# sbrodeur/hierarchical-sparse-coding

Measured on NVIDIA B200. Metric: mp_atoms_per_s, higher is better.
Workload: dtype f32

## Files before the change

### hierarchical_sparse_coding_b200/csrc/engine.cu

```cuda
#include <cuda_runtime.h>
#include <stdio.h>
#include <stdlib.h>
#include <string.h>
#include <math.h>

#include <string>
#include <vector>

#include "../../include/hsc_b200.h"
#include "common.cuh"
#include "correlate_simt.cuh"
#include "correlate_tc.cuh"
#include "pursuit.cuh"
#include "locomp.cuh"
#include "decode.cuh"
#include "ksvd.cuh"
#include "kmeans.cuh"
#include "events.cuh"

using namespace hsc;

namespace {

size_t align_up(size_t v, size_t a = 256) { return (v + a - 1) / a * a; }
// ... 272 lines not shown
    a.has_snr = !isnan(e->opt.tolerance_snr); a.tol_snr = a.has_snr ? (real)e->opt.tolerance_snr : (real)0;
    a.has_scale = !isnan(e->opt.tolerance_residual_scale);
    a.tol_scale = a.has_scale ? (real)e->opt.tolerance_residual_scale : (real)0;
    a.null_thres = (real)e->opt.min_coefficients;
    a.eps = sizeof(real) == 4 ? (real)1.1920928955078125e-07 : (real)2.220446049250313e-16;
    if (e->opt.energy_eps > 0.0) a.eps = (real)e->opt.energy_eps;
    a.coef_mode = e->opt.coef_mode;
    a.max_passes = e->opt.max_passes_per_run;
    a.max_events_total = e->opt.max_events_total;
    a.nb_blocks = e->opt.nb_blocks;
    a.ncand_max = l.ncand_max;
    a.edge_ext = (real*)(e->ws + l.off_edge); a.edge_stride = l.edge_stride;
    a.cand_t = (int*)(e->ws + l.off_cand_t); a.cand_k = (int*)(e->ws + l.off_cand_k); a.cand_c = (real*)(e->ws + l.off_cand_c);
    a.prof = nullptr;
    a.locomp_scratch = nullptr;
    {
        static const char* rr_env = getenv("HSC_RERANK");
        double tol = e->opt.rerank_tolerance < 0.0 ? 4e-6 : e->opt.rerank_tolerance;
        if (rr_env) tol = atof(rr_env);
        a.rerank_tol = sizeof(real) == 4 ? (float)tol : 0.f;
    }
    {
        static const int early = getenv("HSC_K2_EARLY_ISSUE") ? atoi(getenv("HSC_K2_EARLY_ISSUE")) : 0;
        a.early_issue = early > 0 ? 1 : 0;
        static const int nextpf = getenv("HSC_K2_NEXT_PREFETCH") ? atoi(getenv("HSC_K2_NEXT_PREFETCH")) : -1;
        a.next_prefetch = nextpf >= 0 ? (nextpf > 0 ? 1 : 0)
                                      : ((e->K * sizeof(real)) / 16 >= 32 && e->S > 1 && e->S <= 2 * 148 ? 1 : 0);
    }
    static const int prefetch = getenv("HSC_PREFETCH") ? atoi(getenv("HSC_PREFETCH")) : -1;
    a.prefetch = prefetch;
    static const int variant = getenv("HSC_PURSUIT_VARIANT") ? atoi(getenv("HSC_PURSUIT_VARIANT")) : 4;
    static const int tma_mode = getenv("HSC_K2_TMA") ? atoi(getenv("HSC_K2_TMA")) : 1;
    static const int tma_stages_max = getenv("HSC_K2_TMA_STAGES") ? atoi(getenv("HSC_K2_TMA_STAGES")) : 4;
    a.tma_rows = a.tma_stages = a.tma_bytes = 0;
    size_t dyn_smem = 0;
    int rps = 1;
    const size_t row_bytes = (size_t)e->K * sizeof(real);
    const int NW = variant == 6 ? 4 : 8;
    if (tma_mode && variant != 0 && row_bytes % 16 == 0) {
        const int VN = 16 / (int)sizeof(real);
        const int nvec = (int)e->K / VN;
        const int gv = nvec >= 32 ? 32 : pow2_at_least(nvec);
        const int W = 2 * (int)e->L - 1;
        const int rpw = 32 / gv;
        if (variant == 6 && (size_t)NW * 3 * 2 * 2 * rpw * row_bytes <= 48 * 1024 && W >= 2 * NW * 2 * rpw) rps = 2;
        const size_t stage = (size_t)NW * 2 * rpw * rps * row_bytes;
        const int steps = (W + NW * rpw * rps - 1) / (NW * rpw * rps);
        int ns = (int)((48 * 1024) / stage);
        if (ns < 2) ns = (int)((72 * 1024) / stage);
        if (ns < 3 && e->S <= 2 * 148) ns = (int)((100 * 1024) / stage) < 3 ? ns : 3;
        {
            static const int ring_kb = getenv("HSC_K2_RING_KB") ? atoi(getenv("HSC_K2_RING_KB")) : 0;
            if (ring_kb > 0) ns = (int)(((size_t)ring_kb * 1024) / stage);
        }
        if (ns > tma_stages_max) ns = tma_stages_max;
        if (ns > steps) ns = steps;
        if (ns > 32 / NW) ns = 32 / NW;
        if (ns >= 1) {
            a.tma_rows = rpw * rps; a.tma_stages = ns;
            dyn_smem = stage * ns;
            a.tma_bytes = (int)dyn_smem;
// ... 48 lines not shown
            }
        }
        if (!fast) {
            a.tma_rows = a.tma_stages = a.tma_bytes = 0;
            locomp_kernel<real, 128><<<(unsigned)e->S, 128, 0, st>>>(a);
        }
        e->launches++;
        HSC_CUDA(e, cudaGetLastError());
        return HSC_OK;
    }
    static const int smh_mode = getenv("HSC_K2_SMH") ? atoi(getenv("HSC_K2_SMH")) : 1;
    const bool slots_fit = l.n2 <= kSlotMax || (e->S <= 148 && dyn_smem + (size_t)l.n2 * sizeof(unsigned long long) + slot3_bytes <= 200 * 1024);
    const bool smh = (dyn_smem > 0 || tiny_row) && smh_mode && sizeof(real) == 4 && l.G1 == 128 && slots_fit && (l.G1 % 32) == 0 &&
                     (2 * e->L - 1 + l.G1 - 1) / l.G1 + 1 <= kDirtyMax && (long long)l.G1 * e->K < (1ll << 32);
    if (smh) dyn_smem += (size_t)l.n2 * sizeof(unsigned long long) + slot3_bytes;
    {
        static const int smem_kb = getenv("HSC_K2_SMEM_KB") ? atoi(getenv("HSC_K2_SMEM_KB")) : 0;
        if (smem_kb > 0 && dyn_smem > 0 && dyn_smem < (size_t)smem_kb * 1024) dyn_smem = (size_t)smem_kb * 1024;
    }
#define HSC_LAUNCH_K2(NT_, MINB_, VIF_, TMA_, SMH_, RPS_)                                                                        \
    do {                                                                                                                          \
        if (dyn_smem > 0)                                                                                                         \
            HSC_CUDA(e, cudaFuncSetAttribute(pursuit_kernel<real, NT_, MINB_, VIF_, TMA_, SMH_, RPS_>,                            \
                                             cudaFuncAttributeMaxDynamicSharedMemorySize, (int)dyn_smem));                        \
        pursuit_kernel<real, NT_, MINB_, VIF_, TMA_, SMH_, RPS_><<<(unsigned)e->S, NT_, dyn_smem, st>>>(a);                       \
    } while (0)
    switch (variant) {
        case 0:
            HSC_LAUNCH_K2(256, 2, 4, false, false, 1);
            break;
        case 6:
            if (dyn_smem > 0 && smh && rps == 2) HSC_LAUNCH_K2(128, 4, 2, true, true, 2);
            else if (dyn_smem > 0 && smh) HSC_LAUNCH_K2(128, 4, 2, true, true, 1);
            else if (dyn_smem > 0 && rps == 2) HSC_LAUNCH_K2(128, 4, 2, true, false, 2);
            else if (dyn_smem > 0) HSC_LAUNCH_K2(128, 4, 2, true, false, 1);
            else HSC_LAUNCH_K2(128, 4, 2, false, false, 1);
            break;
        default:
            if (tiny_row && smh) HSC_LAUNCH_K2(256, 4, 2, false, true, 1);
            else if (dyn_smem > 0 && smh) HSC_LAUNCH_K2(256, 4, 2, true, true, 1);
            else if (dyn_smem > 0) HSC_LAUNCH_K2(256, 4, 2, true, false, 1);
            else HSC_LAUNCH_K2(256, 4, 2, false, false, 1);
            break;
    }
#undef HSC_LAUNCH_K2
    e->launches++;
    HSC_CUDA(e, cudaGetLastError());
#ifdef HSC_PROFILE_PHASES
    {
        std::vector<long long> h((size_t)e->S * 16);
        cudaStreamSynchronize(st);
        cudaMemcpy(h.data(), a.prof, h.size() * sizeof(long long), cudaMemcpyDeviceToHost);
        double tot[8] = {0, 0, 0, 0, 0, 0, 0, 0};
        for (long long i = 0; i < e->S; ++i) for (int j = 0; j < 8; ++j) tot[j] += (double)h[(size_t)i * 16 + j];
// ... 850 lines not shown
```

### hierarchical_sparse_coding_b200/csrc/pursuit.cuh

```cuda
#pragma once
#include <limits.h>
#include "common.cuh"

namespace hsc {

template <typename real>
struct MpArgs {
    int T, K, L, F, off;
    int G1, n2, G2, n3;
    const real* D;
    const real* G;
    const real* w;
    real* map;
    real* resid;
    real* val1; int* idx1;
    real* val2; int* idx2;
    real* val3; int* idx3;
    unsigned* bitmap;
    long long bitmap_words;
    hsc_signal_state* state;
    int* ev_pos; int* ev_idx; real* ev_coef;
    long long cap;
    long long max_nnz;
    real tol_snr; int has_snr;
// ... 6 lines not shown
    int nb_blocks;
    int ncand_max;
    int* cand_t; int* cand_k; real* cand_c;
    double* locomp_scratch;
    real* edge_ext;
    long long edge_stride;
    int prefetch;
    int tma_rows, tma_stages;
    int tma_bytes;
    long long* prof;
    int scalar_window;
    int row32;
    int next_prefetch;
    int early_issue;
    float rerank_tol;
};

__device__ __forceinline__ unsigned long long pack_key(float v, int row_local, int k, int K) {
    const unsigned vb = __float_as_uint(v);
    return vb == 0u ? 0ull : (((unsigned long long)vb << 32) | (unsigned long long)(0xFFFFFFFFu - (unsigned)(row_local * K + k)));
}
__device__ __forceinline__ unsigned long long pack_key(double, int, int, int) { return 0ull; }

__device__ __forceinline__ unsigned lds_u32(uint32_t saddr) {
    unsigned v;
    asm("ld.shared.u32 %0, [%1];" : "=r"(v) : "r"(saddr));
    return v;
}

__device__ __forceinline__ unsigned long long warp_max_u64(unsigned long long key) {
// ... 422 lines not shown
                cur_key = 0ull;
            }
            cur_key = key > cur_key ? key : cur_key;
        }
        gmap += gstep;
        ggram += gstep;
        trow += NW;
        s = (s + 1 == NS) ? 0 : s + 1;
    }
    if constexpr (SMH) {
        if (lane == 0 && cur_key) atomicMax(&dirty[cur_g - glo], cur_key);
    }
    return phase;
}

template <typename real, int NT>
__device__ __noinline__ void edge_recorrelate(const MpArgs<real>& a, real* map_s, const real* ext, int ext_row0, int ra, int rb) {
    const int K = a.K, F = a.F, LF = a.L * a.F;
    constexpr int R = 8, U = 8;
    constexpr int KPT = NT <= 128 ? 2 : 1;
    const int kt = K < NT ? K : NT;
    const int ngroups = NT / kt;
    const int grp = threadIdx.x / kt;
    if (grp >= ngroups) return;
    const int nchunks = (rb - ra + 1 + R - 1) / R;
    for (int kk = threadIdx.x - grp * kt; kk < K; kk += KPT * kt) {
        const real* dd[KPT];
#pragma unroll
        for (int p = 0; p < KPT; ++p) dd[p] = a.D + (long long)min(kk + p * kt, K - 1) * LF;
        for (int c = grp; c < nchunks; c += ngroups) {
// ... 125 lines not shown

template <typename real>
__device__ __forceinline__ double exact_score_warp(const MpArgs<real>& a, const hsc_signal_state& st, const real* map_s, const real* res_s,
                                                   int r, int k) {
    double sc;
    const bool overhang = (r < a.off) || (r > a.T - a.L + a.off);
    if (!overhang || !overhang_row_written(st, r, a.off, a.T, a.L)) sc = fabs(residual_dot_warp<real>(a, res_s, r, k));
    else sc = fabs((double)__ldcg(map_s + (long long)r * a.K + k));
    return a.w ? sc * fabs((double)a.w[k]) : sc;
}

constexpr int kRerankMax = 32;

template <typename real, typename Lvl2>
__device__ __forceinline__ void rerank_candidates(const MpArgs<real>& a, const hsc_signal_state& st, const real* map_s, const real* res_s,
                                                  const real* v1, Lvl2 lvl2, uint32_t slot3_saddr, int g1s, real thr, int& t_out, int& k_out) {
    __shared__ int cand_g[kRerankMax], cand_r[kRerankMax], cand_k[kRerankMax];
    const int lane = threadIdx.x & 31;
    const int T = a.T, K = a.K, L = a.L, F = a.F, LF = a.L * a.F;
    int ng = 0;
    if (slot3_saddr) {
        const int n3 = (a.n2 + 31) >> 5;
        for (int b0 = 0; b0 < n3; b0 += 32) {
            const int b = b0 + lane;
            unsigned mb = __ballot_sync(0xffffffffu, b < n3 && (real)__uint_as_float(lds_u32(slot3_saddr + 4u * (unsigned)b)) >= thr);
            while (mb) {
                const int g = ((b0 + __ffs(mb) - 1) << 5) + lane;
                mb &= mb - 1;
                const bool h = g < a.n2 && lvl2(g) >= thr;
                const unsigned m = __ballot_sync(0xffffffffu, h);
                if (h) { const int slot = ng + __popc(m & ((1u << lane) - 1u)); if (slot < kRerankMax) cand_g[slot] = g; }
// ... 23 lines not shown
            for (int u = 0; u < 4; ++u) { const int r = rb + u * 32 + lane; h[u] = r < r_end && v1[r] >= thr; }
#pragma unroll
            for (int u = 0; u < 4; ++u) {
                const unsigned m = __ballot_sync(0xffffffffu, h[u]);
                if (h[u]) { const int slot = nr + __popc(m & ((1u << lane) - 1u)); if (slot < kRerankMax) cand_r[slot] = rb + u * 32 + lane; }
                nr += __popc(m);
            }
        }
    }
    nr = min(nr, kRerankMax);
    __syncwarp();
    int nc = 0;
    for (int i = 0; i < nr; ++i) {
        const int rr = cand_r[i];
        const real* mrow = map_s + (long long)rr * K;
        for (int kb = 0; kb < K; kb += 128) {
            bool h[4];
#pragma unroll
            for (int u = 0; u < 4; ++u) {
                const int kk = kb + u * 32 + lane;
                h[u] = false;
                if (kk < K) { const real m = __ldcg(mrow + kk); h[u] = rabs<real>(a.w ? m * a.w[kk] : m) >= thr; }
            }
#pragma unroll
            for (int u = 0; u < 4; ++u) {
                const unsigned m = __ballot_sync(0xffffffffu, h[u]);
                if (h[u]) {
                    const int slot = nc + __popc(m & ((1u << lane) - 1u));
                    if (slot < kRerankMax) { cand_g[slot] = rr; cand_k[slot] = kb + u * 32 + lane; }
                }
                nc += __popc(m);
            }
        }
    }
    nc = min(nc, kRerankMax);
    __syncwarp();
    const int sub = lane >> 3, sl = lane & 7;
// ... 29 lines not shown
        }
        for (int m = 16; m >= 8; m >>= 1) {
            const double os = __shfl_xor_sync(0xffffffffu, sc, m);
            const long long of = __shfl_xor_sync(0xffffffffu, flat, m);
            if (os > sc || (os == sc && of < flat)) { sc = os; flat = of; }
        }
        if (sc > best || (sc == best && flat < best_flat)) { best = sc; best_flat = flat; }
    }
    if (best_flat != LLONG_MAX && best >= 0.0) {
        t_out = (int)(best_flat / K);
        k_out = (int)(best_flat - (long long)t_out * K);
    }
}

template <typename real>
__device__ __forceinline__ bool near_tie_in_group(const MpArgs<real>& a, const real* map_s, const real* v1, int g1s, int t, int k, real thr) {
    const int lane = threadIdx.x & 31;
    bool amb = false;
    const int r0 = (t >> g1s) << g1s, r1 = min(r0 + (1 << g1s), a.T);
    const real* mrow = map_s + (long long)t * a.K;
    constexpr int RU = 4, MU = 8;
    real vv[RU], mm[MU];
#pragma unroll
    for (int u = 0; u < RU; ++u) { const int r = r0 + lane + 32 * u; vv[u] = r < r1 ? v1[r] : (real)-1; }
#pragma unroll
    for (int u = 0; u < MU; ++u) { const int kk = lane + 32 * u; mm[u] = kk < a.K ? __ldcg(mrow + kk) : (real)0; }
#pragma unroll
    for (int u = 0; u < RU; ++u) { const int r = r0 + lane + 32 * u; amb |= r < r1 && r != t && vv[u] >= thr; }
    for (int r = r0 + lane + 32 * RU; r < r1; r += 32) amb |= (r != t) && (v1[r] >= thr);
#pragma unroll
    for (int u = 0; u < MU; ++u) {
        const int kk = lane + 32 * u;
        amb |= kk < a.K && (kk != k) && (rabs<real>(a.w ? mm[u] * a.w[kk] : mm[u]) >= thr);
    }
    for (int kk = lane + 32 * MU; kk < a.K; kk += 32) {
        const real m = __ldcg(mrow + kk);
        amb |= (kk != k) && (rabs<real>(a.w ? m * a.w[kk] : m) >= thr);
    }
    return __any_sync(0xffffffffu, amb);
}

template <typename real, bool SMH>
__device__ __noinline__ real near_tie_watch(const MpArgs<real>& a, hsc_signal_state& st, const real* map_s, const real* res_s,
                                            const real* v1, const int* i1, const real* v2g, const real* v3g, const int* i3g, int g1s,
                                            int t, int k, real vbest, real second, uint32_t slot2_saddr, int next_g) {
    const int lane = threadIdx.x & 31;
    if constexpr (!SMH) {
        real bv = (real)0;
        int bt = INT_MAX;
        for (int e = lane; e < a.n3; e += 32) take_first_max(bv, bt, v3g[e], i3g[e]);
        group_argmax(bv, bt, 32);
        if (bt == INT_MAX) return (real)-1;
        t = bt;
        k = i1[t];
        vbest = bv;
    }
    if (st.reserved == 0) {
        __syncwarp();
        if (lane == 0) st.reserved = (int)__float_as_uint((float)vbest);
        __syncwarp();
    }
    const real thr = vbest - (real)a.rerank_tol * (vbest + (real)__uint_as_float((unsigned)st.reserved));
    bool amb;
    if constexpr (SMH) {
        amb = second >= thr;
    } else {
        const int gsel = t >> g1s;
        amb = false;
        for (int e = lane; e < a.n2; e += 32) amb |= (e != gsel) && (v2g[e] >= thr);
        amb = __any_sync(0xffffffffu, amb);
    }
    if (!amb) amb = near_tie_in_group<real>(a, map_s, v1, g1s, t, k, thr);
    if constexpr (SMH) {
        if (a.next_prefetch && next_g < 0 && second > (real)0) {
            const unsigned sbits = __float_as_uint((float)second);
            const uint32_t slot3_saddr = slot2_saddr + 8u * (unsigned)a.n2;
            const int n3 = (a.n2 + 31) >> 5;
            int bb = INT_MAX;
            for (int e = lane; e < n3; e += 32)
                if (lds_u32(slot3_saddr + 4u * (unsigned)e) == sbits && e != ((t >> g1s) >> 5)) bb = min(bb, e);
            bb = __reduce_min_sync(0xffffffffu, bb);
            if (bb != INT_MAX) {
                const int g = (bb << 5) + lane;
                const unsigned ghi = g < a.n2 ? lds_u32(slot2_saddr + 8u * (unsigned)g + 4u) : 0u;
                const int gg = __reduce_min_sync(0xffffffffu, ghi == sbits ? g : INT_MAX);
                if (gg != INT_MAX) next_g = gg;
            }
// ... 14 lines not shown
            } else {
                const int r0 = next_g << g1s;
                p = v1 + r0;
                bytes = (unsigned)(min(r0 + (1 << g1s), a.T) - r0) * sizeof(real);
            }
            if ((((unsigned long long)p) & 15ull) == 0 && (bytes & 15u) == 0 && bytes > 0)
                asm volatile("cp.async.bulk.prefetch.L2.global [%0], %1;" :: "l"(p), "r"(bytes) : "memory");
        }
    }
    return amb ? thr : (real)-1;
}

template <typename real, bool SMH>
__device__ __noinline__ real near_tie_resolve(const MpArgs<real>& a, hsc_signal_state& st, const real* map_s, const real* res_s,
                                              const real* v1, uint32_t slot2_saddr, const real* v2g, int g1s, real thr,
                                              int& t, int& k) {
    if constexpr (SMH) {
        auto lvl2 = [&](int g) { return (real)__uint_as_float(lds_u32(slot2_saddr + 8u * (unsigned)g + 4u)); };
        rerank_candidates<real>(a, st, map_s, res_s, v1, lvl2, slot2_saddr + 8u * (unsigned)a.n2, g1s, thr, t, k);
    } else {
        auto lvl2 = [&](int g) { return v2g[g]; };
        rerank_candidates<real>(a, st, map_s, res_s, v1, lvl2, 0u, g1s, thr, t, k);
    }
    const bool row_overhangs = (t < a.off) || (t > a.T - a.L + a.off);
    const bool from_residual = a.coef_mode == 1 && (!row_overhangs || !overhang_row_written(st, t, a.off, a.T, a.L));
    return from_residual ? (real)residual_dot_warp<real>(a, res_s, t, k) : __ldcg(map_s + (long long)t * a.K + k);
}

template <typename real, int NT>
__device__ __noinline__ int build_pass_list(const MpArgs<real>& a, const real* map_s, const real* res_s, const real* v1,
                                            const int* i1, int* ct, int* ck, real* cc, int offset_flag, double energy_signal) {
    const int T = a.T, K = a.K, L = a.L, F = a.F, off = a.off, LF = L * F;
    const int tid = threadIdx.x, lane = tid & 31, warp = tid >> 5, nwarps = NT >> 5;
    __shared__ int s_count;
    int bs = a.nb_blocks < 0 ? 4 * L : (int)floor((double)T / (double)a.nb_blocks);
    if (bs & 1) bs += 1;
    int nblk = (T + bs - 1) / bs;
// ... 132 lines not shown
        out[4] = g2 == INT_MAX ? -1 : g2;
    }
    __threadfence_block();
}

__device__ __forceinline__ void refold_block(const unsigned long long* slot2, unsigned* slot3, int b, int n2) {
    const int g = (b << 5) + (int)(threadIdx.x & 31);
    const unsigned hi = g < n2 ? (unsigned)(slot2[g] >> 32) : 0u;
    const unsigned mx = __reduce_max_sync(0xffffffffu, hi);
    if ((threadIdx.x & 31) == 0) slot3[b] = mx;
}

constexpr int kSlotMax = 1024;
constexpr int kDirtyMax = 8;

template <typename real, int NT, int MINB, int VIF, bool TMA, bool SMH, int RPS = 1>
__global__ void __launch_bounds__(NT, MINB) pursuit_kernel(MpArgs<real> a) {
    const int s = blockIdx.x;
    const int tid = threadIdx.x, lane = tid & 31, warp = tid >> 5;
    constexpr int NW = NT / 32;
    const int T = a.T, K = a.K, L = a.L, F = a.F, off = a.off;
    const int W = 2 * L - 1;
    const int LF = L * F;
#ifdef HSC_PROFILE_PHASES
    long long prof_kernel_t0;
    { unsigned long long ns_; asm volatile("mov.u64 %0, %%globaltimer;" : "=l"(ns_)); prof_kernel_t0 = (long long)ns_; }
#endif

    struct Ctx {
        real* map_s; real* res_s; real* v1; int* i1; real* v2; int* i2; real* v3; int* i3;
        unsigned* bits; int* evp; int* evi; real* evc;
        int* ct; int* ck; real* cc;
// ... 35 lines not shown
        real coef;
        real thr;
    } sel;
    __shared__ double red_a[NW], red_b[NW];
    __shared__ real red_m[NW];
    __shared__ struct { int t, k; unsigned vbest, second; int g2; } watch;

    extern __shared__ __align__(128) unsigned char win_smem[];
    __shared__ __align__(8) unsigned long long win_bar[(NT / 32) * 4];
    constexpr bool tma_on = TMA;
    unsigned win_phase = 0;
    unsigned long long* slot2 = reinterpret_cast<unsigned long long*>(win_smem + a.tma_bytes);
    unsigned* slot3 = reinterpret_cast<unsigned*>(slot2 + a.n2);
    __shared__ unsigned long long dirty_slot[kDirtyMax];
    const int g1s = 31 - __clz(a.G1);
    if (tid == 0) {
        st = a.state[s];
        if (tma_on) {
            for (int i = 0; i < (NT / 32) * a.tma_stages; ++i) mbarrier_init(smem_addr_u32(&win_bar[i]), 1);
            asm volatile("fence.mbarrier_init.release.cluster;" ::: "memory");
            fence_proxy_async_all();
        }
    }
    __syncthreads();
    if (st.status != HSC_RUNNING && st.status != HSC_PAUSE_CAPACITY && st.status != HSC_PAUSE_PASSES) return;

    const int g = min(32, pow2_at_least(K));
    const int ngroups = NT / g;
    const int grp = tid / g, lig = tid % g;
    constexpr int VN = VecOf<real>::N;
// ... 38 lines not shown
            st.initialised = 1;
        }
        if constexpr (!SMH) {
            rekey_level<real>(v1, nullptr, T, v2, i2, 0, a.n2 - 1, a.G1, NT);
            __syncthreads();
            rekey_level<real>(v2, i2, a.n2, v3, i3, 0, a.n3 - 1, a.G2, NT);
            __syncthreads();
        }
    }
    if constexpr (SMH) {
        if (tid < kDirtyMax) dirty_slot[tid] = 0ull;
        for (int gi = warp; gi < a.n2; gi += NW) {
            unsigned long long best = 0ull;
            const int e1 = min((gi + 1) << g1s, T);
            for (int r = (gi << g1s) + lane; r < e1; r += 32) {
                const unsigned long long key = pack_key(v1[r], r & (a.G1 - 1), i1[r], K);
                best = key > best ? key : best;
            }
            best = warp_max_u64(best);
            if (lane == 0) slot2[gi] = best;
        }
        __syncthreads();
        for (int b = warp; b < (a.n2 + 31) >> 5; b += NW) refold_block(slot2, slot3, b, a.n2);
    }
    if (tid == 0) {
        st.status = HSC_RUNNING;
        st.n_buffered = 0;
    }
    __syncthreads();

    long long passes_this_run = 0;
    const bool rerank_on = sizeof(real) == 4 && a.rerank_tol > 0.f && a.nb_blocks == 1;
#ifdef HSC_PROFILE_PHASES
    long long prof_t = clock64(), prof_acc[8] = {0, 0, 0, 0, 0, 0, 0, 0};
    long long prof_edge[4] = {0, 0, 0, 0};
    long long prof_loop_t0;
    { unsigned long long ns_; asm volatile("mov.u64 %0, %%globaltimer;" : "=l"(ns_)); prof_loop_t0 = (long long)ns_; }
#define HSC_STAMP(i) do { if (tid == 0) { long long now_ = clock64(); prof_acc[i] += now_ - prof_t; prof_t = now_; } } while (0)
#else
#define HSC_STAMP(i) do { } while (0)
#endif
    while (true) {
        HSC_STAMP(0);
        if (st.n_buffered >= a.cap) {
            if (tid == 0) st.status = HSC_PAUSE_CAPACITY;
            break;
        }
        const bool block_mode = a.nb_blocks != 1;
        const bool new_pass = !block_mode || st.pass_cursor >= st.pass_count;
        if (new_pass && a.max_passes > 0 && passes_this_run >= a.max_passes) {
            if (tid == 0) st.status = HSC_PAUSE_PASSES;
            break;
        }
        if (block_mode && new_pass) {
            const int n = build_pass_list<real, NT>(a, map_s, res_s, v1, i1, cx.ct, cx.ck, cx.cc, st.offset_flag, st.energy_signal);
            if (tid == 0) {
                st.pass_count = n;
                st.pass_cursor = 0;
            }
            __syncthreads();
            if (n == 0) {
                if (tid == 0) {
                    st.passes += 1;
                    st.status = HSC_STOP_EMPTY;
                }
// ... 64 lines not shown
            if constexpr (SMH) {
                asm volatile("bar.sync 1, 64;" ::: "memory");
                if (watch.t >= 0)
                    thr = near_tie_watch<real, true>(a, st, map_s, res_s, v1, i1, v2, v3, i3, g1s, watch.t, watch.k,
                                                     (real)__uint_as_float(watch.vbest), (real)__uint_as_float(watch.second),
                                                     smem_addr_u32(slot2), watch.g2);
            } else {
                thr = near_tie_watch<real, false>(a, st, map_s, res_s, v1, i1, v2, v3, i3, g1s, 0, 0, (real)0, (real)-1, 0u, -1);
            }
            if (lane == 0) sel.thr = thr;
        }
        __syncthreads();
        if (rerank_on && sel.thr >= (real)0) {
            if (warp == 0) {
                int t = sel.t, k = sel.k;
                const real coef = near_tie_resolve<real, SMH>(a, st, map_s, res_s, v1, smem_addr_u32(slot2), v2, g1s, sel.thr, t, k);
                __syncwarp();
                if (lane == 0) {
                    sel.t = t;
                    sel.k = k;
                    sel.edge = (t - (L - 1) < off) || (t + (L - 1) > T - L + off);
                    sel.coef = coef;
                    st.reranked += 1;
                }
            }
            __syncthreads();
        }
        HSC_STAMP(1);
        const int t = sel.t, k = sel.k, edge = sel.edge;
        const real coef = sel.coef;
        const bool pass_ends = sel.last != 0;

        const bool is_null = (a.null_thres >= (real)0) ? !(rabs<real>(coef) > a.null_thres) : (coef == (real)0);
        if (!block_mode && is_null) {
            if (tid == 0) {
                st.passes += 1;
                st.status = HSC_STOP_EMPTY;
            }
            break;
        }

        if constexpr (TMA) {
            if (!edge && a.early_issue) gram_window_issue<real, NT, RPS>(K, L, map_s, a.G + (long long)k * W * K, t, gv, win_smem, win_bar, a.tma_stages);
        }

        unsigned bk_old = 0u, bk_m = 0u;
        if (tid == 0) {
            const unsigned long long bit = (unsigned long long)t * K + k;
            bk_m = 1u << (bit & 31);
            bk_old = atomicOr(bits + (bit >> 5), bk_m);
            evp[st.n_buffered] = t;
            evi[st.n_buffered] = k;
            evc[st.n_buffered] = coef;
            st.n_buffered += 1;
            st.n_events += 1;
        }
        HSC_STAMP(5);

// ... 4 lines not shown
        const int jhi = (sstart + L > T) ? (T - sstart) : L;
        const real* dd = a.D + (long long)k * LF;
        real* rr = res_s + (long long)sstart * F;
        const int q_first = jlo * F + tid;
        real ro_first = (real)0, dq_first = (real)0;
        if (q_first < jhi * F) {
            ro_first = rr[q_first];
            dq_first = dd[q_first];
        }

        if constexpr (SMH) {
            const int span0 = g2_lo << g1s, span1 = min((g2_hi + 1) << g1s, T);
            for (int r0 = span0 + warp * 32; r0 < span1; r0 += NT) {
                const int r = r0 + lane;
                unsigned long long key = 0ull;
                if (r < span1 && (r < row_lo || r > row_hi)) key = pack_key(v1[r], r & (a.G1 - 1), i1[r], K);
                key = warp_max_u64(key);
                if (lane == 0 && key) atomicMax(&dirty_slot[(r0 >> g1s) - g2_lo], key);
            }
        }

        {
            double eb = 0.0, ea = 0.0;
            if (q_first < jhi * F) {
                const real rn = sub_scaled(ro_first, coef, dq_first);
                rr[q_first] = rn;
                eb = fma((double)ro_first, (double)ro_first, eb);
                ea = fma((double)rn, (double)rn, ea);
            }
            for (int q = q_first + NT; q < jhi * F; q += NT) {
                real ro = rr[q];
// ... 2 lines not shown
                eb = fma((double)ro, (double)ro, eb);
                ea = fma((double)rn, (double)rn, ea);
            }
            eb = warp_sum(eb);
            ea = warp_sum(ea);
            if (lane == 0) {
                red_b[warp] = eb;
                red_a[warp] = ea;
            }
        }
        HSC_STAMP(6);

        if (!edge) {
            const real* Gk = a.G + (long long)k * W * K;
            if constexpr (TMA) {
                if (!a.early_issue) gram_window_issue<real, NT, RPS>(K, L, map_s, Gk, t, gv, win_smem, win_bar, a.tma_stages);
                if (a.w) win_phase = gram_update_tma<real, NT, true, SMH, RPS>(K, L, a.w, map_s, Gk, v1, i1, t, coef, gv, win_smem, win_bar, a.tma_stages, win_phase, dirty_slot, g2_lo, g1s, true);
                else if (RPS == 1 && gv == 32 && a.row32) win_phase = gram_update_row32<real, NT, SMH>(K, L, map_s, Gk, v1, i1, t, coef, win_smem, win_bar, a.tma_stages, win_phase, dirty_slot, g2_lo, g1s);
                else win_phase = gram_update_tma<real, NT, false, SMH, RPS>(K, L, a.w, map_s, Gk, v1, i1, t, coef, gv, win_smem, win_bar, a.tma_stages, win_phase, dirty_slot, g2_lo, g1s, true);
            }
            else if (!(SMH && !TMA) && vec_pv == 1 && !a.w && !a.scalar_window) gram_update_vec<real, 1, NT, VIF, false>(K, L, a.w, map_s, Gk, v1, i1, t, coef, gv);
            else if (!(SMH && !TMA) && vec_pv == 2 && !a.w && !a.scalar_window) gram_update_vec<real, 2, NT, VIF, false>(K, L, a.w, map_s, Gk, v1, i1, t, coef, gv);
            else if (!(SMH && !TMA) && vec_pv == 4 && VIF >= 4 && !a.w && !a.scalar_window) gram_update_vec<real, 4, NT, VIF, false>(K, L, a.w, map_s, Gk, v1, i1, t, coef, gv);
            else {
                for (int base = 0; base < W; base += ngroups) {
                    const int i = base + grp;
                    const bool valid = i < W;
                    real bv = (real)0;
                    int bi = INT_MAX;
                    const int tr = t - (L - 1) + i;
                    if (valid) {
                        real* mrow = map_s + (long long)tr * K;
                        const real* grow = Gk + (long long)i * K;
                        for (int kk = lig; kk < K; kk += g) {
// ... 71 lines not shown
                    slot2[g2_lo + lane] = dirty_slot[lane];
                    dirty_slot[lane] = 0ull;
                }
                __syncwarp();
                for (int b = g2_lo >> 5; b <= g2_hi >> 5; ++b) refold_block(slot2, slot3, b, a.n2);
            }
        } else {
            rekey_level<real>(v1, nullptr, T, v2, i2, g2_lo, g2_hi, a.G1, NT);
        }
        if (tid == 0) {
            double eb = 0.0, ea = 0.0;
            for (int i = 0; i < NW; ++i) {
                eb += red_b[i];
                ea += red_a[i];
            }
            if (bk_old & bk_m) st.duplicates += 1;
            else st.nnz += 1;
            const real loss = (real)eb - (real)ea;
            const real e_now = (real)st.energy_residual - loss;
            st.energy_residual = (double)e_now;
            if (block_mode) st.pass_cursor += 1;
            int stop = 0;
            if (e_now < a.eps) {
                stop = HSC_STOP_ENERGY;
            } else {
                const real snr = (real)10 * rlog10<real>((real)st.energy_signal / e_now);
                if (a.max_nnz >= 0 && st.nnz >= a.max_nnz) stop = HSC_STOP_NNZ;
                else if (a.has_snr && snr >= a.tol_snr) stop = HSC_STOP_SNR;
                else if (a.max_events_total > 0 && st.n_events >= a.max_events_total) stop = HSC_STOP_MAX_EVENTS;
            }
// ... 57 lines not shown
#undef HSC_STAMP
#undef map_s
#undef res_s
#undef v1
#undef i1
#undef v2
#undef i2
#undef v3
#undef i3
#undef bits
#undef evp
#undef evi
#undef evc
}

}
```

Baseline: 10.30 million.

## Add lazy read-only correlation map path deferring interior Gram updates via event log

Adds a lazy pursuit kernel variant in which interior map rows are no longer written back after each atom selection. Selected atoms are logged, and when a window is loaded their contributions are reapplied on the fly through an extra TMA-loaded Gram row, plus direct loads for further overlapping events. Only band rows near the signal edges are stored. The log is flushed to global memory when there are too many overlaps or when the run pauses, and runner-up values are saved so tie detection still works. The aim is to remove per-iteration global write-back traffic, at the cost of extra Gram reads, a larger staging ring and considerable added complexity.

```diff
diff --git a/hierarchical_sparse_coding_b200/csrc/engine.cu b/hierarchical_sparse_coding_b200/csrc/engine.cu
--- a/hierarchical_sparse_coding_b200/csrc/engine.cu
+++ b/hierarchical_sparse_coding_b200/csrc/engine.cu
@@ -310,6 +310,8 @@
     a.cand_t = (int*)(e->ws + l.off_cand_t); a.cand_k = (int*)(e->ws + l.off_cand_k); a.cand_c = (real*)(e->ws + l.off_cand_c);
     a.prof = nullptr;
     a.locomp_scratch = nullptr;
+    a.lazy = 0;
+    a.runner = (unsigned*)(e->ws + l.off_keys);
     {
         static const char* rr_env = getenv("HSC_RERANK");
         double tol = e->opt.rerank_tolerance < 0.0 ? 4e-6 : e->opt.rerank_tolerance;
@@ -333,6 +335,11 @@
     int rps = 1;
     const size_t row_bytes = (size_t)e->K * sizeof(real);
     const int NW = variant == 6 ? 4 : 8;
+    const char* ro_env = getenv("HSC_K2_READONLY_MAP");
+    const bool lazy_shape = (!ro_env || atoi(ro_env) != 0) && sizeof(real) == 4 && e->opt.method == 0 && variant == 4 && tma_mode && !(e->opt.use_weights && e->w_dev) &&
+                            e->opt.nb_blocks == 1 && e->opt.coef_mode == 1 && e->T <= 65536 && (e->K * sizeof(real)) / 16 >= 32 &&
+                            (size_t)e->K * (2 * e->L - 1) * e->K * sizeof(real) <= 64ull * 1024 * 1024;
+    const int stage_rows = lazy_shape ? 3 : 2;
     if (tma_mode && variant != 0 && row_bytes % 16 == 0) {
         const int VN = 16 / (int)sizeof(real);
         const int nvec = (int)e->K / VN;
@@ -340,7 +347,7 @@
         const int W = 2 * (int)e->L - 1;
         const int rpw = 32 / gv;
         if (variant == 6 && (size_t)NW * 3 * 2 * 2 * rpw * row_bytes <= 48 * 1024 && W >= 2 * NW * 2 * rpw) rps = 2;
-        const size_t stage = (size_t)NW * 2 * rpw * rps * row_bytes;
+        const size_t stage = (size_t)NW * stage_rows * rpw * rps * row_bytes;
         const int steps = (W + NW * rpw * rps - 1) / (NW * rpw * rps);
         int ns = (int)((48 * 1024) / stage);
         if (ns < 2) ns = (int)((72 * 1024) / stage);
@@ -419,6 +426,10 @@
     const bool smh = (dyn_smem > 0 || tiny_row) && smh_mode && sizeof(real) == 4 && l.G1 == 128 && slots_fit && (l.G1 % 32) == 0 &&
                      (2 * e->L - 1 + l.G1 - 1) / l.G1 + 1 <= kDirtyMax && (long long)l.G1 * e->K < (1ll << 32);
     if (smh) dyn_smem += (size_t)l.n2 * sizeof(unsigned long long) + slot3_bytes;
+    if (lazy_shape && smh && a.row32 && a.tma_stages >= 1 && (size_t)a.tma_bytes >= (size_t)kLazyLogCap * 8 && l.n2 <= kSlotMax) {
+        a.lazy = 1;
+        dyn_smem += kLazySmemBytes;
+    }
     {
         static const int smem_kb = getenv("HSC_K2_SMEM_KB") ? atoi(getenv("HSC_K2_SMEM_KB")) : 0;
         if (smem_kb > 0 && dyn_smem > 0 && dyn_smem < (size_t)smem_kb * 1024) dyn_smem = (size_t)smem_kb * 1024;
@@ -442,7 +453,12 @@
             else HSC_LAUNCH_K2(128, 4, 2, false, false, 1);
             break;
         default:
-            if (tiny_row && smh) HSC_LAUNCH_K2(256, 4, 2, false, true, 1);
+            if (a.lazy && sizeof(real) == 4) {
+                const MpArgs<float>& af = reinterpret_cast<const MpArgs<float>&>(a);
+                HSC_CUDA(e, cudaFuncSetAttribute(pursuit_kernel_ro<256, 4>, cudaFuncAttributeMaxDynamicSharedMemorySize, (int)dyn_smem));
+                pursuit_kernel_ro<256, 4><<<(unsigned)e->S, 256, dyn_smem, st>>>(af);
+            }
+            else if (tiny_row && smh) HSC_LAUNCH_K2(256, 4, 2, false, true, 1);
             else if (dyn_smem > 0 && smh) HSC_LAUNCH_K2(256, 4, 2, true, true, 1);
             else if (dyn_smem > 0) HSC_LAUNCH_K2(256, 4, 2, true, false, 1);
             else HSC_LAUNCH_K2(256, 4, 2, false, false, 1);
diff --git a/hierarchical_sparse_coding_b200/csrc/pursuit.cuh b/hierarchical_sparse_coding_b200/csrc/pursuit.cuh
--- a/hierarchical_sparse_coding_b200/csrc/pursuit.cuh
+++ b/hierarchical_sparse_coding_b200/csrc/pursuit.cuh
@@ -44,6 +44,8 @@
     int next_prefetch;
     int early_issue;
     float rerank_tol;
+    int lazy;
+    unsigned* runner;
 };
 
 __device__ __forceinline__ unsigned long long pack_key(float v, int row_local, int k, int K) {
@@ -496,6 +498,286 @@
     return phase;
 }
 
+constexpr int kLazyBand = 3;
+constexpr int kLazyLogCap = 768;
+constexpr int kLazyOvMax = 16;
+constexpr int kLazySmemBytes = 16 + kLazyLogCap * 2 + kLazyOvMax * 16;
+constexpr int kLazyRebuilt = (int)0x80000000;
+
+struct LazyState { int n, m; long long base; };
+
+__device__ __forceinline__ bool lazy_band_row(int r, int T, int L) { return r < kLazyBand * L || r >= T - kLazyBand * L; }
+
+struct LazyPtrs {
+    unsigned short* log; int* ov_p; int* ov_k; float* ov_c;
+    const int* evp; const int* evi; const float* evc;
+    float* map_s; unsigned* runner; unsigned char* ring;
+    __device__ __forceinline__ LazyPtrs(const MpArgs<float>& a, const LazyState& lz) {
+        extern __shared__ __align__(128) unsigned char win_smem[];
+        const long long s = blockIdx.x;
+        unsigned char* mem = reinterpret_cast<unsigned char*>(
+            (reinterpret_cast<unsigned long long>(win_smem + a.tma_bytes + 8 * a.n2 + 4 * ((a.n2 + 31) >> 5)) + 15ull) & ~15ull);
+        log = reinterpret_cast<unsigned short*>(mem);
+        ov_p = reinterpret_cast<int*>(mem + 2 * kLazyLogCap);
+        ov_k = ov_p + kLazyOvMax;
+        ov_c = reinterpret_cast<float*>(ov_k + kLazyOvMax);
+        evp = a.ev_pos + s * a.cap + lz.base;
+        evi = a.ev_idx + s * a.cap + lz.base;
+        evc = a.ev_coef + s * a.cap + lz.base;
+        map_s = a.map + s * a.T * a.K;
+        runner = a.runner + 2ll * s * a.T;
+        ring = win_smem;
+    }
+    __device__ __forceinline__ int pos(int j) const { return j < kLazyLogCap ? (int)log[j] : __ldcg(evp + j); }
+};
+
+__device__ __noinline__ void lazy_overlaps(const MpArgs<float>& a, LazyState& lz, int t) {
+    const LazyPtrs P(a, lz);
+    const int lane = threadIdx.x & 31;
+    const int n = lz.n, L = a.L;
+    int m = 0;
+    for (int j0 = 0; j0 < n; j0 += 32) {
+        const int j = j0 + lane;
+        const int p = j < n ? P.pos(j) : INT_MIN / 2;
+        const bool hit = abs(p - t) <= 2 * L - 2;
+        const unsigned mask = __ballot_sync(0xffffffffu, hit);
+        if (hit) {
+            const int slot = m + __popc(mask & ((1u << lane) - 1u));
+            if (slot < kLazyOvMax) { P.ov_p[slot] = p; P.ov_k[slot] = j; }
+        }
+        m += __popc(mask);
+    }
+    if (m > kLazyOvMax) m = -1;
+    __syncwarp();
+    if (lane < m) {
+        const int j = P.ov_k[lane];
+        P.ov_k[lane] = P.evi[j];
+        P.ov_c[lane] = P.evc[j];
+    }
+    if (lane == 0) lz.m = m;
+    __syncwarp();
+}
+
+template <int NT>
+__device__ __noinline__ void lazy_flush(const MpArgs<float>& a, LazyState& lz) {
+    const LazyPtrs P(a, lz);
+    const int K = a.K, L = a.L, T = a.T, n = lz.n;
+    constexpr int U = 4;
+    const int chunk = a.tma_bytes / 12;
+    int* sk = reinterpret_cast<int*>(P.ring);
+    float* sc = reinterpret_cast<float*>(sk + chunk);
+    int* sp = reinterpret_cast<int*>(sc + chunk);
+    const int W = 2 * L - 1;
+    const int nvec = K / 4;
+    float4* map4 = reinterpret_cast<float4*>(P.map_s);
+    const float4* G4 = reinterpret_cast<const float4*>(a.G);
+    for (int i = 0; i < n; ++i) {
+        if (i % chunk == 0) {
+            for (int e = threadIdx.x; e < chunk && i + e < n; e += NT) { sk[e] = P.evi[i + e]; sc[e] = P.evc[i + e]; sp[e] = P.pos(i + e); }
+            __syncthreads();
+        }
+        const int ic = i % chunk;
+        const int p = sp[ic];
+        const int lo = max(p - (L - 1), kLazyBand * L), hi = min(p + (L - 1), T - kLazyBand * L - 1);
+        const float nc = -sc[ic];
+        const long long gbase = ((long long)sk[ic] * W + (lo - p + (L - 1))) * nvec;
+        const int nv = (hi - lo + 1) * nvec;
+        for (int e0 = threadIdx.x; e0 < nv; e0 += U * NT) {
+            float4 m[U], g[U];
+#pragma unroll
+            for (int u = 0; u < U; ++u) {
+                const int e = e0 + u * NT;
+                if (e < nv) {
+                    m[u] = __ldcg(map4 + (long long)lo * nvec + e);
+                    g[u] = __ldg(G4 + gbase + e);
+                }
+            }
+#pragma unroll
+            for (int u = 0; u < U; ++u) {
+                const int e = e0 + u * NT;
+                if (e < nv) {
+                    m[u].x = fmaf(nc, g[u].x, m[u].x); m[u].y = fmaf(nc, g[u].y, m[u].y);
+                    m[u].z = fmaf(nc, g[u].z, m[u].z); m[u].w = fmaf(nc, g[u].w, m[u].w);
+                    __stcg(map4 + (long long)lo * nvec + e, m[u]);
+                }
+            }
+        }
+        __syncthreads();
+    }
+    fence_proxy_async_all();
+    if (threadIdx.x == 0) { lz.base += lz.n; lz.n = 0; lz.m = 0; }
+    __syncthreads();
+}
+
+__device__ __noinline__ const float* lazy_rebuild_row(const MpArgs<float>& a, const LazyState& lz, int r) {
+    const LazyPtrs P(a, lz);
+    float* buf = reinterpret_cast<float*>(P.ring);
+    const int lane = threadIdx.x & 31;
+    const int K = a.K, L = a.L, n = lz.n;
+    const int W = 2 * L - 1;
+    for (int kk = lane; kk < K; kk += 32) buf[kk] = __ldcg(P.map_s + (long long)r * K + kk);
+    for (int j0 = 0; j0 < n; j0 += 32) {
+        const int j = j0 + lane;
+        const int pj = j < n ? P.pos(j) : INT_MIN / 2;
+        unsigned mask = __ballot_sync(0xffffffffu, abs(pj - r) <= L - 1);
+        while (mask) {
+            const int src = __ffs(mask) - 1;
+            mask &= mask - 1;
+            const int jj = j0 + src;
+            const int p = __shfl_sync(0xffffffffu, pj, src);
+            const float nc = -P.evc[jj];
+            const float* g = a.G + ((long long)P.evi[jj] * W + (r - p + (L - 1))) * K;
+            for (int kk = lane; kk < K; kk += 32) buf[kk] = fmaf(nc, __ldg(g + kk), buf[kk]);
+        }
+    }
+    __syncwarp();
+    return buf;
+}
+
+template <int NT>
+__device__ __noinline__ unsigned gram_update_row32_ro(const MpArgs<float>& a, const LazyState& lz, const float* Gk_in, int t_in, float coef,
+                                                      unsigned long long* bars, unsigned phase, unsigned long long* dirty, int glo) {
+    constexpr int NW = NT / 32;
+    const LazyPtrs P(a, lz);
+    const int K = a.K, L = a.L, T = a.T, NS = a.tma_stages, m = lz.m;
+    const int g1s = 31 - __clz(a.G1);
+    float* map_s = P.map_s;
+    float* __restrict__ v1 = a.val1 + (long long)blockIdx.x * T;
+    int* __restrict__ i1 = a.idx1 + (long long)blockIdx.x * T;
+    const int* ov_p = P.ov_p; const int* ov_k = P.ov_k; const float* ov_c = P.ov_c;
+    const int lane = threadIdx.x & 31;
+    const int warp = __shfl_sync(0xffffffffu, (int)(threadIdx.x >> 5), 0);
+    const int t = __shfl_sync(0xffffffffu, t_in, 0);
+    const float* Gk = reinterpret_cast<const float*>(__shfl_sync(0xffffffffu, reinterpret_cast<unsigned long long>(Gk_in), 0));
+    const int W = 2 * L - 1;
+    const int nvec = K / 4;
+    const float ncoef = -coef;
+    const uint32_t row_bytes = (uint32_t)(K * sizeof(float));
+    const uint32_t stage_bytes = 3u * row_bytes;
+    unsigned char* wsm = P.ring + (size_t)warp * NS * stage_bytes;
+    const uint32_t wsm_u = smem_addr_u32(wsm);
+    const uint32_t bar_u = smem_addr_u32(bars + warp * NS);
+    const int nsteps = warp < W ? (W - warp + NW - 1) / NW : 0;
+    const int trow0 = t - (L - 1) + warp;
+    const float4* G4 = reinterpret_cast<const float4*>(a.G);
+    auto first_cover = [&](int r) {
+        if (lazy_band_row(r, T, L)) return -1;
+        for (int q = 0; q < m; ++q)
+            if (abs(ov_p[q] - r) <= L - 1) return q;
+        return -1;
+    };
+    auto issue = [&](int jj, int s) {
+        const int r = trow0 + jj * NW;
+        const int q = first_cover(r);
+        const uint32_t bar = bar_u + 8u * (uint32_t)s;
+        const uint32_t dst = wsm_u + (uint32_t)s * stage_bytes;
+        mbarrier_expect_tx(bar, (q >= 0 ? 3u : 2u) * row_bytes);
+        bulk_load_g2s(dst, map_s + (long long)r * K, row_bytes, bar);
+        bulk_load_g2s(dst + row_bytes, Gk + (long long)(r - t + (L - 1)) * K, row_bytes, bar);
+        if (q >= 0) bulk_load_g2s(dst + 2u * row_bytes, a.G + ((long long)ov_k[q] * W + (r - ov_p[q] + (L - 1))) * K, row_bytes, bar);
+    };
+    if (elect_one_sync())
+        for (int j = 0; j < NS && j < nsteps; ++j) issue(j, j);
+    int trow = trow0;
+    int s = 0;
+    int cur_g = -1;
+    unsigned long long cur_key = 0ull;
+#pragma unroll 1
+    for (int j = 0; j < nsteps; ++j) {
+        const uint32_t bar = bar_u + 8u * (uint32_t)s;
+        mbarrier_wait_parity(bar, (phase >> s) & 1u);
+        phase ^= 1u << s;
+        unsigned char* stg = wsm + (size_t)s * stage_bytes;
+        float4* mrow = reinterpret_cast<float4*>(stg);
+        const float4* grow = reinterpret_cast<const float4*>(stg + row_bytes);
+        const float4* xrow = reinterpret_cast<const float4*>(stg + 2u * row_bytes);
+        const bool band = lazy_band_row(trow, T, L);
+        const int q0 = first_cover(trow);
+        const float nc0 = q0 >= 0 ? -ov_c[q0] : 0.f;
+        float bv = 0.f, s2 = 0.f;
+        int bi = INT_MAX;
+#pragma unroll 2
+        for (int v = lane; v < nvec; v += 32) {
+            float pm[4], pg[4];
+            unpack(mrow[v], pm);
+            if (q0 >= 0) {
+                unpack(xrow[v], pg);
+#pragma unroll
+                for (int c = 0; c < 4; ++c) pm[c] = fmaf(nc0, pg[c], pm[c]);
+#pragma unroll 1
+                for (int q = q0 + 1; q < m; ++q) {
+                    const int d = trow - ov_p[q];
+                    if (d < -(L - 1) || d > L - 1) continue;
+                    unpack(__ldg(G4 + ((long long)ov_k[q] * W + d + (L - 1)) * nvec + v), pg);
+                    const float nc = -ov_c[q];
+#pragma unroll
+                    for (int c = 0; c < 4; ++c) pm[c] = fmaf(nc, pg[c], pm[c]);
+                }
+            }
+            unpack(grow[v], pg);
+#pragma unroll
+            for (int c = 0; c < 4; ++c) {
+                pm[c] = fmaf(ncoef, pg[c], pm[c]);
+                const float x = fabsf(pm[c]);
+                if (x > bv) { s2 = bv; bv = x; bi = v * 4 + c; }
+                else s2 = fmaxf(s2, x);
+            }
+            if (band) mrow[v] = pack(pm, float4());
+        }
+        fence_proxy_async_smem();
+        __syncwarp();
+        if (elect_one_sync()) {
+            if (band) {
+                bulk_store_s2g(map_s + (long long)trow * K, wsm_u + (uint32_t)s * stage_bytes, row_bytes);
+                bulk_commit();
+            }
+            if (j + NS < nsteps) {
+                if (band) bulk_wait_read_all();
+                issue(j + NS, s);
+            }
+        }
+        const int my_bi = bi;
+        const float my_bv = bv;
+        group_argmax(bv, bi, 32);
+        if (!band) {
+            const unsigned rb = __reduce_max_sync(0xffffffffu, __float_as_uint(my_bi == bi ? s2 : my_bv));
+            if (lane == 0) P.runner[2ll * trow] = rb;
+        }
+        if (lane == 0) {
+            v1[trow] = bv;
+            i1[trow] = band ? bi : (bi | kLazyRebuilt);
+        }
+        const unsigned long long key = pack_key(bv, trow & ((1 << g1s) - 1), bi, K);
+        const int gg = trow >> g1s;
+        if (gg != cur_g) {
+            if (lane == 0 && cur_key) atomicMax(&dirty[cur_g - glo], cur_key);
+            cur_g = gg;
+            cur_key = 0ull;
+        }
+        cur_key = key > cur_key ? key : cur_key;
+        trow += NW;
+        s = (s + 1 == NS) ? 0 : s + 1;
+    }
+    if (lane == 0 && cur_key) atomicMax(&dirty[cur_g - glo], cur_key);
+    return phase;
+}
+
+template <int NT>
+__device__ __noinline__ unsigned lazy_window(const MpArgs<float>& a, LazyState& lz, int t, int k, float coef, unsigned long long* bars,
+                                             unsigned phase, unsigned long long* dirty, int glo) {
+    __syncthreads();
+    if (lz.m < 0) lazy_flush<NT>(a, lz);
+    return gram_update_row32_ro<NT>(a, lz, a.G + (long long)k * (2 * a.L - 1) * a.K, t, coef, bars, phase, dirty, glo);
+}
+
+template <int NT>
+__device__ __noinline__ void lazy_pause(const MpArgs<float>& a, LazyState& lz) { lazy_flush<NT>(a, lz); }
+
+__device__ __forceinline__ void lazy_append(const MpArgs<float>& a, LazyState& lz, int t) {
+    if (lz.n < kLazyLogCap) LazyPtrs(a, lz).log[lz.n] = (unsigned short)t;
+    lz.n += 1;
+}
+
 template <typename real, int NT>
 __device__ __noinline__ void edge_recorrelate(const MpArgs<real>& a, real* map_s, const real* ext, int ext_row0, int ra, int rb) {
     const int K = a.K, F = a.F, LF = a.L * a.F;
@@ -651,7 +933,8 @@
 
 template <typename real, typename Lvl2>
 __device__ __forceinline__ void rerank_candidates(const MpArgs<real>& a, const hsc_signal_state& st, const real* map_s, const real* res_s,
-                                                  const real* v1, Lvl2 lvl2, uint32_t slot3_saddr, int g1s, real thr, int& t_out, int& k_out) {
+                                                  const real* v1, Lvl2 lvl2, uint32_t slot3_saddr, int g1s, real thr, int& t_out, int& k_out,
+                                                  const LazyState* lz) {
     __shared__ int cand_g[kRerankMax], cand_r[kRerankMax], cand_k[kRerankMax];
     const int lane = threadIdx.x & 31;
     const int T = a.T, K = a.K, L = a.L, F = a.F, LF = a.L * a.F;
@@ -705,13 +988,15 @@
     for (int i = 0; i < nr; ++i) {
         const int rr = cand_r[i];
         const real* mrow = map_s + (long long)rr * K;
+        const bool rebuilt = lz != nullptr && !lazy_band_row(rr, T, L);
+        const float* buf = rebuilt ? lazy_rebuild_row(reinterpret_cast<const MpArgs<float>&>(a), *lz, rr) : nullptr;
         for (int kb = 0; kb < K; kb += 128) {
             bool h[4];
 #pragma unroll
             for (int u = 0; u < 4; ++u) {
                 const int kk = kb + u * 32 + lane;
                 h[u] = false;
-                if (kk < K) { const real m = __ldcg(mrow + kk); h[u] = rabs<real>(a.w ? m * a.w[kk] : m) >= thr; }
+                if (kk < K) { const real m = rebuilt ? (real)buf[kk] : __ldcg(mrow + kk); h[u] = rabs<real>(a.w ? m * a.w[kk] : m) >= thr; }
             }
 #pragma unroll
             for (int u = 0; u < 4; ++u) {
@@ -771,13 +1056,16 @@
 }
 
 template <typename real>
-__device__ __forceinline__ bool near_tie_in_group(const MpArgs<real>& a, const real* map_s, const real* v1, int g1s, int t, int k, real thr) {
+__device__ __forceinline__ bool near_tie_in_group(const MpArgs<real>& a, const real* map_s, const real* v1, const int* i1, const unsigned* runner,
+                                                  int g1s, int t, int k, real thr) {
     const int lane = threadIdx.x & 31;
     bool amb = false;
     const int r0 = (t >> g1s) << g1s, r1 = min(r0 + (1 << g1s), a.T);
     const real* mrow = map_s + (long long)t * a.K;
     constexpr int RU = 4, MU = 8;
     real vv[RU], mm[MU];
+    const int it = runner ? i1[t] : 0;
+    const unsigned rbits = runner ? runner[2ll * t] : 0u;
 #pragma unroll
     for (int u = 0; u < RU; ++u) { const int r = r0 + lane + 32 * u; vv[u] = r < r1 ? v1[r] : (real)-1; }
 #pragma unroll
@@ -785,6 +1073,7 @@
 #pragma unroll
     for (int u = 0; u < RU; ++u) { const int r = r0 + lane + 32 * u; amb |= r < r1 && r != t && vv[u] >= thr; }
     for (int r = r0 + lane + 32 * RU; r < r1; r += 32) amb |= (r != t) && (v1[r] >= thr);
+    if (it & kLazyRebuilt) return __any_sync(0xffffffffu, amb || (real)__uint_as_float(rbits) >= thr);
 #pragma unroll
     for (int u = 0; u < MU; ++u) {
         const int kk = lane + 32 * u;
@@ -801,6 +1090,7 @@
 __device__ __noinline__ real near_tie_watch(const MpArgs<real>& a, hsc_signal_state& st, const real* map_s, const real* res_s,
                                             const real* v1, const int* i1, const real* v2g, const real* v3g, const int* i3g, int g1s,
                                             int t, int k, real vbest, real second, uint32_t slot2_saddr, int next_g) {
+    const unsigned* runner = a.lazy ? a.runner + 2ll * blockIdx.x * a.T : nullptr;
     const int lane = threadIdx.x & 31;
     if constexpr (!SMH) {
         real bv = (real)0;
@@ -827,7 +1117,7 @@
         for (int e = lane; e < a.n2; e += 32) amb |= (e != gsel) && (v2g[e] >= thr);
         amb = __any_sync(0xffffffffu, amb);
     }
-    if (!amb) amb = near_tie_in_group<real>(a, map_s, v1, g1s, t, k, thr);
+    if (!amb) amb = near_tie_in_group<real>(a, map_s, v1, i1, runner, g1s, t, k, thr);
     if constexpr (SMH) {
         if (a.next_prefetch && next_g < 0 && second > (real)0) {
             const unsigned sbits = __float_as_uint((float)second);
@@ -872,13 +1162,13 @@
 template <typename real, bool SMH>
 __device__ __noinline__ real near_tie_resolve(const MpArgs<real>& a, hsc_signal_state& st, const real* map_s, const real* res_s,
                                               const real* v1, uint32_t slot2_saddr, const real* v2g, int g1s, real thr,
-                                              int& t, int& k) {
+                                              int& t, int& k, const LazyState* lz) {
     if constexpr (SMH) {
         auto lvl2 = [&](int g) { return (real)__uint_as_float(lds_u32(slot2_saddr + 8u * (unsigned)g + 4u)); };
-        rerank_candidates<real>(a, st, map_s, res_s, v1, lvl2, slot2_saddr + 8u * (unsigned)a.n2, g1s, thr, t, k);
+        rerank_candidates<real>(a, st, map_s, res_s, v1, lvl2, slot2_saddr + 8u * (unsigned)a.n2, g1s, thr, t, k, lz);
     } else {
         auto lvl2 = [&](int g) { return v2g[g]; };
-        rerank_candidates<real>(a, st, map_s, res_s, v1, lvl2, 0u, g1s, thr, t, k);
+        rerank_candidates<real>(a, st, map_s, res_s, v1, lvl2, 0u, g1s, thr, t, k, lz);
     }
     const bool row_overhangs = (t < a.off) || (t > a.T - a.L + a.off);
     const bool from_residual = a.coef_mode == 1 && (!row_overhangs || !overhang_row_written(st, t, a.off, a.T, a.L));
@@ -1041,8 +1331,8 @@
 constexpr int kSlotMax = 1024;
 constexpr int kDirtyMax = 8;
 
-template <typename real, int NT, int MINB, int VIF, bool TMA, bool SMH, int RPS = 1>
-__global__ void __launch_bounds__(NT, MINB) pursuit_kernel(MpArgs<real> a) {
+template <typename real, int NT, int VIF, bool TMA, bool SMH, int RPS, bool LAZY>
+__device__ __forceinline__ void pursuit_body(const MpArgs<real>& a) {
     const int s = blockIdx.x;
     const int tid = threadIdx.x, lane = tid & 31, warp = tid >> 5;
     constexpr int NW = NT / 32;
@@ -1108,6 +1398,9 @@
     unsigned* slot3 = reinterpret_cast<unsigned*>(slot2 + a.n2);
     __shared__ unsigned long long dirty_slot[kDirtyMax];
     const int g1s = 31 - __clz(a.G1);
+    __shared__ LazyState lz;
+    const MpArgs<float>& af = reinterpret_cast<const MpArgs<float>&>(a);
+    constexpr bool lazy = LAZY && SMH && TMA && sizeof(real) == 4;
     if (tid == 0) {
         st = a.state[s];
         if (tma_on) {
@@ -1176,7 +1469,7 @@
             unsigned long long best = 0ull;
             const int e1 = min((gi + 1) << g1s, T);
             for (int r = (gi << g1s) + lane; r < e1; r += 32) {
-                const unsigned long long key = pack_key(v1[r], r & (a.G1 - 1), i1[r], K);
+                const unsigned long long key = pack_key(v1[r], r & (a.G1 - 1), lazy ? i1[r] & ~kLazyRebuilt : i1[r], K);
                 best = key > best ? key : best;
             }
             best = warp_max_u64(best);
@@ -1188,6 +1481,7 @@
     if (tid == 0) {
         st.status = HSC_RUNNING;
         st.n_buffered = 0;
+        lz.n = 0; lz.m = 0; lz.base = 0;
     }
     __syncthreads();
 
@@ -1205,12 +1499,14 @@
     while (true) {
         HSC_STAMP(0);
         if (st.n_buffered >= a.cap) {
+            if constexpr (lazy) lazy_pause<NT>(af, lz);
             if (tid == 0) st.status = HSC_PAUSE_CAPACITY;
             break;
         }
         const bool block_mode = a.nb_blocks != 1;
         const bool new_pass = !block_mode || st.pass_cursor >= st.pass_count;
         if (new_pass && a.max_passes > 0 && passes_this_run >= a.max_passes) {
+            if constexpr (lazy) lazy_pause<NT>(af, lz);
             if (tid == 0) st.status = HSC_PAUSE_PASSES;
             break;
         }
@@ -1305,7 +1601,8 @@
         if (rerank_on && sel.thr >= (real)0) {
             if (warp == 0) {
                 int t = sel.t, k = sel.k;
-                const real coef = near_tie_resolve<real, SMH>(a, st, map_s, res_s, v1, smem_addr_u32(slot2), v2, g1s, sel.thr, t, k);
+                const real coef = near_tie_resolve<real, SMH>(a, st, map_s, res_s, v1, smem_addr_u32(slot2), v2, g1s, sel.thr, t, k,
+                                                              lazy ? &lz : nullptr);
                 __syncwarp();
                 if (lane == 0) {
                     sel.t = t;
@@ -1332,7 +1629,11 @@
         }
 
         if constexpr (TMA) {
-            if (!edge && a.early_issue) gram_window_issue<real, NT, RPS>(K, L, map_s, a.G + (long long)k * W * K, t, gv, win_smem, win_bar, a.tma_stages);
+            if (!edge && a.early_issue && !lazy) gram_window_issue<real, NT, RPS>(K, L, map_s, a.G + (long long)k * W * K, t, gv, win_smem, win_bar, a.tma_stages);
+        }
+
+        if constexpr (lazy) {
+            if (!edge && warp == 2) lazy_overlaps(af, lz, t);
         }
 
         unsigned bk_old = 0u, bk_m = 0u;
@@ -1367,7 +1668,7 @@
             for (int r0 = span0 + warp * 32; r0 < span1; r0 += NT) {
                 const int r = r0 + lane;
                 unsigned long long key = 0ull;
-                if (r < span1 && (r < row_lo || r > row_hi)) key = pack_key(v1[r], r & (a.G1 - 1), i1[r], K);
+                if (r < span1 && (r < row_lo || r > row_hi)) key = pack_key(v1[r], r & (a.G1 - 1), lazy ? i1[r] & ~kLazyRebuilt : i1[r], K);
                 key = warp_max_u64(key);
                 if (lane == 0 && key) atomicMax(&dirty_slot[(r0 >> g1s) - g2_lo], key);
             }
@@ -1400,10 +1701,14 @@
         if (!edge) {
             const real* Gk = a.G + (long long)k * W * K;
             if constexpr (TMA) {
+                if constexpr (lazy) {
+                    win_phase = lazy_window<NT>(af, lz, t, k, (float)coef, win_bar, win_phase, dirty_slot, g2_lo);
+                } else {
                 if (!a.early_issue) gram_window_issue<real, NT, RPS>(K, L, map_s, Gk, t, gv, win_smem, win_bar, a.tma_stages);
                 if (a.w) win_phase = gram_update_tma<real, NT, true, SMH, RPS>(K, L, a.w, map_s, Gk, v1, i1, t, coef, gv, win_smem, win_bar, a.tma_stages, win_phase, dirty_slot, g2_lo, g1s, true);
                 else if (RPS == 1 && gv == 32 && a.row32) win_phase = gram_update_row32<real, NT, SMH>(K, L, map_s, Gk, v1, i1, t, coef, win_smem, win_bar, a.tma_stages, win_phase, dirty_slot, g2_lo, g1s);
                 else win_phase = gram_update_tma<real, NT, false, SMH, RPS>(K, L, a.w, map_s, Gk, v1, i1, t, coef, gv, win_smem, win_bar, a.tma_stages, win_phase, dirty_slot, g2_lo, g1s, true);
+                }
             }
             else if (!(SMH && !TMA) && vec_pv == 1 && !a.w && !a.scalar_window) gram_update_vec<real, 1, NT, VIF, false>(K, L, a.w, map_s, Gk, v1, i1, t, coef, gv);
             else if (!(SMH && !TMA) && vec_pv == 2 && !a.w && !a.scalar_window) gram_update_vec<real, 2, NT, VIF, false>(K, L, a.w, map_s, Gk, v1, i1, t, coef, gv);
@@ -1505,6 +1810,7 @@
                 eb += red_b[i];
                 ea += red_a[i];
             }
+            if constexpr (lazy) lazy_append(af, lz, t);
             if (bk_old & bk_m) st.duplicates += 1;
             else st.nnz += 1;
             const real loss = (real)eb - (real)ea;
@@ -1592,4 +1898,10 @@
 #undef evc
 }
 
-}
+template <typename real, int NT, int MINB, int VIF, bool TMA, bool SMH, int RPS = 1>
+__global__ void __launch_bounds__(NT, MINB) pursuit_kernel(MpArgs<real> a) { pursuit_body<real, NT, VIF, TMA, SMH, RPS, false>(a); }
+
+template <int NT, int MINB>
+__global__ void __launch_bounds__(NT, MINB) pursuit_kernel_ro(MpArgs<float> a) { pursuit_body<float, NT, 2, true, true, 1, true>(a); }
+
+}
```

New measurement: 6.999 million, median of 6. 32.1% lower.
